# DefaultRui/VLN-VER

Hardware: AMD Instinct MI355X
Metric: viewpoints/sec (multi-view->voxel fwd+bwd), vocc.py config (higher is better)
Workload: dtype bf16

## Files before the change

vln-ver_amd/csrc/ver_gemm.hip:

```cpp
#include "ver_gemm_tile.h"

namespace {
using namespace gemm_tile;
constexpr int kStageBytes = 32768;
constexpr int kStages = 4;
constexpr int kLdsBytes = kStages * kStageBytes;

struct TapArgs {
    const __bf16* lattice;
    long lattice_bytes;
    int B, H, W, C, ntaps, P;
    const float* rowpos;
    const __bf16* cst;
    long cst_bytes;
    int CW, ncst;
    unsigned desc[64];
    long plane_elems;
};

struct GemmArgs {
    const __bf16* A;
    const __bf16* W;
    const float* bias;
    __bf16* C;
// ... 31 lines not shown
    asm volatile("s_load_dword %0, %1, %2" : "=s"(v) : "s"(ts.tab), "s"(idx * 4) : "memory");
    return v;
}
__device__ __forceinline__ void desc_ready(unsigned& d) { asm volatile("s_waitcnt lgkmcnt(0)" : "+s"(d) : : "memory"); }

template <int L>
__device__ __forceinline__ void tap_begin(const TapArgs& t, TapLane& tl, TapWave& ts, unsigned d, __amdgpu_buffer_rsrc_t& ra,
                                          __amdgpu_buffer_rsrc_t rcst) {
    const bool live = ts.tap < t.ntaps;
    const bool is_cst = live && (d >> 31) != 0;
    const int dx = (int)(d << 24) >> 24, dy = (int)(d << 16) >> 24, dz = (int)(d >> 16) & 63, pl = (int)(d >> 22) & 63;
    int o1 = kOutside, o2 = kOutside, seglen = 2 * t.C;
    if (is_cst) {
        seglen = 2 * t.CW;
        if (tl.b1 >= 0) o1 = (tl.pos1 * t.ncst + dz) * t.CW * 2 + tl.chunk;
        if (tl.b2 >= 0) o2 = (tl.pos2 * t.ncst + dz) * t.CW * 2 + tl.chunk;
        ra = rcst;
    } else if (live) {
        const LatticeGeom geom = {t.B, t.H, t.W, t.C};
        const int c1 = cell_off<L>(geom, tl.b1, tl.zl1, tl.y1 + dy, tl.x1 + dx, dz);
        const int c2 = cell_off<L>(geom, tl.b2, tl.zl2, tl.y2 + dy, tl.x2 + dx, dz);
        if (c1 != kOutside) o1 = c1 + tl.chunk;
        if (c2 != kOutside) o2 = c2 + tl.chunk;
        ra = __builtin_amdgcn_make_buffer_rsrc((void*)(t.lattice + (long)pl * t.plane_elems), 0,
                                               (int)max(0L, min(t.lattice_bytes, 0x7FFFFFFFL)), 0x00020000);
    }
    ts.seglen = seglen;
    tl.vo1 = o1;
    tl.vo2 = o2;
}

template <int IMPL, bool PRO>
__device__ __forceinline__ void request_a(char* dst, const GemmLane& c, __amdgpu_buffer_rsrc_t& ra, __amdgpu_buffer_rsrc_t rcst,
                                          int& soA, const TapArgs& t, TapLane& tl, TapWave& ts) {
    if constexpr (IMPL < 0) {
        __builtin_amdgcn_raw_ptr_buffer_load_lds(ra, (lds_void*)dst, 16, c.voA, soA, 0, 0);
        __builtin_amdgcn_raw_ptr_buffer_load_lds(ra, (lds_void*)(dst + 1024), 16, c.voA, soA + c.stepA16, 0, 0);
        soA += 64;
    } else {
        __builtin_amdgcn_raw_ptr_buffer_load_lds(ra, (lds_void*)dst, 16, tl.vo1, ts.ch, 0, 0);
        __builtin_amdgcn_raw_ptr_buffer_load_lds(ra, (lds_void*)(dst + 1024), 16, tl.vo2, ts.ch, 0, 0);
        ts.ch += 64;
        if (ts.ch == ts.seglen) {
            ts.ch = 0;
            ts.tap += 1;
            const unsigned d = ts.next;
            ts.next = desc_load(ts, min(ts.tap + 1, t.ntaps - 1));
            if constexpr (PRO) desc_ready(ts.next);
            tap_begin<IMPL>(t, tl, ts, d, ra, rcst);
        }
    }
}

template <int ST, int IMPL>
__device__ __forceinline__ void phase(char* lds, f32x4 (&acc)[8][4], const GemmLane& c, __amdgpu_buffer_rsrc_t& ra,
                                      __amdgpu_buffer_rsrc_t rw, int& soA, int& soW, const TapArgs& t, TapLane& tl, TapWave& ts,
                                      __amdgpu_buffer_rsrc_t rcst) {
    constexpr int SB = (ST & 1) * kStageBytes;
    constexpr int UP = ST >= 2 ? 65536 : 0;
    const int a0 = c.offA0 + UP;
    i32x4 av[8];
    i32x2 bl[4], bh[4];
    av[0] = row_read<SB>(a0);
    av[1] = row_read<SB + 1024>(a0);
#pragma unroll
    for (int q = 0; q < 4; ++q) {
        const int b = c.offB[q] + UP;
        bl[q] = tr_read<SB + 16384>(b);
        bh[q] = tr_read<SB + 16384 + 512>(b);
        if (q == 0) av[2] = row_read<SB + 2048>(a0), av[3] = row_read<SB + 3072>(a0);
        if (q == 1) av[4] = row_read<SB + 4096>(a0), av[5] = row_read<SB + 5120>(a0);
        if (q == 2) av[6] = row_read<SB + 6144>(a0), av[7] = row_read<SB + 7168>(a0);
    }
    constexpr int DS = ((ST + 2) % kStages) * kStageBytes;
    request_a<IMPL, false>(lds + DS + c.dmaA, c, ra, rcst, soA, t, tl, ts);
    __builtin_amdgcn_raw_ptr_buffer_load_lds(rw, (lds_void*)(lds + DS + 16384 + c.dmaW), 16, c.voW, soW, 0, 0);
    __builtin_amdgcn_raw_ptr_buffer_load_lds(rw, (lds_void*)(lds + DS + 24576 + c.dmaW), 16, c.voW, soW + c.stepW, 0, 0);
    soW += 2 * c.stepW;
    asm volatile("s_waitcnt vmcnt(4)" ::: "memory");
    __builtin_amdgcn_s_barrier();
    asm volatile("s_waitcnt lgkmcnt(0)"
                 : "+v"(av[0]), "+v"(av[1]), "+v"(av[2]), "+v"(av[3]), "+v"(av[4]), "+v"(av[5]), "+v"(av[6]), "+v"(av[7]), "+v"(bl[0]),
                   "+v"(bh[0]), "+v"(bl[1]), "+v"(bh[1]), "+v"(bl[2]), "+v"(bh[2]), "+v"(bl[3]), "+v"(bh[3])
                 :
                 : "memory");
    if constexpr (IMPL >= 0) asm volatile("" : "+s"(ts.next));
    bf16x8 a[8], b[4];
#pragma unroll
    for (int i = 0; i < 8; ++i) a[i] = __builtin_bit_cast(bf16x8, av[i]);
#pragma unroll
    for (int j = 0; j < 4; ++j) b[j] = frag(bl[j], bh[j]);
    __builtin_amdgcn_sched_barrier(0);
    __builtin_amdgcn_s_setprio(1);
#pragma unroll
    for (int it = 0; it < 8; ++it)
#pragma unroll
        for (int jt = 0; jt < 4; ++jt) acc[it][jt] = __builtin_amdgcn_mfma_f32_16x16x32_bf16(a[it], b[jt], acc[it][jt], 0, 0, 0);
    __builtin_amdgcn_s_setprio(0);
    __builtin_amdgcn_sched_barrier(0);
    __builtin_amdgcn_s_barrier();
}


template <int IMPL>
__global__ __launch_bounds__(512) void k_gemm_nn(GemmArgs p) {
    extern __shared__ __attribute__((aligned(1024))) char lds[];
    const int tid = threadIdx.x, lane = tid & 63;
    const int wave = __builtin_amdgcn_readfirstlane(tid >> 6);
    const int wr = wave >> 2, wc = wave & 3;
    const int item = (int)(blockIdx.x & 7) * p.per_xcd + (int)(blockIdx.x >> 3);
    if ((int)(blockIdx.x >> 3) >= p.per_xcd || item >= p.T * p.S) return;
    const int split = item / p.T, tile = item - split * p.T;
    const int mt = tile / p.tiles_n, nt = tile - mt * p.tiles_n;
    const long row0 = (long)mt * kTile;
    const int k0 = split * p.Kc, klen = min(p.Kc, p.K - k0);
    const int nphase = klen / 32;

    const __bf16* ab = IMPL < 0 ? p.A + row0 * p.lda + k0 : p.t.lattice;
    const long abytes = IMPL < 0 ? ((p.M - row0 - 1) * p.lda + klen) * 2 : p.t.lattice_bytes;
    __amdgpu_buffer_rsrc_t ra = __builtin_amdgcn_make_buffer_rsrc((void*)ab, 0, (int)max(0L, min(abytes, 0xFFFFFFFFL)), 0x00020000);
    const __amdgpu_buffer_rsrc_t rcst = __builtin_amdgcn_make_buffer_rsrc((void*)(IMPL < 0 ? ab : p.t.cst), 0,
                                                                          (int)(IMPL < 0 ? 0L : max(0L, min(p.t.cst_bytes, 0x7FFFFFFFL))), 0x00020000);
    const __bf16* wb = p.W + (long)k0 * p.ldw + (long)nt * kTile;
    const long wbytes = ((long)(klen - 1) * p.ldw + p.N - (long)nt * kTile) * 2;
    const __amdgpu_buffer_rsrc_t rw = __builtin_amdgcn_make_buffer_rsrc((void*)wb, 0, (int)max(0L, min(wbytes, 0xFFFFFFFFL)), 0x00020000);
    GemmLane c;
    {
        const int prow = 32 * wave + (lane >> 2);
        const int pch = (lane & 3) ^ Shape::swz_a(prow & 15);
        c.voA = (int)(prow * p.lda * 2) + pch * 16;
        c.dmaA = wave * 2048;
        c.stepA16 = (int)(16 * p.lda * 2);
        const int wrow = lane >> 3, wch = (lane & 7) ^ Shape::swz(wrow, wave >> 2);
        c.voW = (int)(((8 * (wave >> 2) + wrow) * p.ldw + 64 * (wave & 3)) * 2) + wch * 16;
        c.stepW = (int)(16 * p.ldw * 2);
        c.dmaW = wave * 1024;
    }
    {
        const int lbase = (int)(uintptr_t)(__attribute__((address_space(3))) char*)lds;
        const int i = lane & 15, g = lane >> 4;
        c.offA0 = lbase + (128 * wr + i) * 64 + ((g ^ Shape::swz_a(i)) << 4);
#pragma unroll
        for (int q = 0; q < 4; ++q) {
            const int ch = (2 * q + ((i & 3) >> 1)) ^ Shape::swz(i >> 2, g & 1);
            c.offB[q] = lbase + (g >> 1) * 8192 + (g & 1) * 4096 + (i >> 2) * 128 + ch * 16 + (i & 1) * 8 + wc * 1024;
        }
    }
    TapLane tl = {};
    TapWave ts = {};
    if constexpr (IMPL >= 0) {
        const int prow = 32 * wave + (lane >> 2);
        const int hw = p.t.H * p.t.W;
        auto decode = [&](long r, int& b, int& zl, int& y, int& x) {
            if (r >= p.M) {
                b = -1, zl = y = x = 0;
                return;
            }
            b = (int)(r / p.t.P);
            const int pos = (int)(r - (long)b * p.t.P);
            zl = pos / hw;
            const int rem = pos - zl * hw;
            y = rem / p.t.W;
            x = rem - y * p.t.W;
        };
        decode(row0 + prow, tl.b1, tl.zl1, tl.y1, tl.x1);
        decode(row0 + prow + 16, tl.b2, tl.zl2, tl.y2, tl.x2);
        tl.pos1 = (tl.zl1 * p.t.H + tl.y1) * p.t.W + tl.x1;
        tl.pos2 = (tl.zl2 * p.t.H + tl.y2) * p.t.W + tl.x2;
        tl.chunk = ((lane & 3) ^ Shape::swz_a(prow & 15)) * 16;
        ts.tab = (const __attribute__((address_space(4))) unsigned*)((const __attribute__((address_space(4))) char*)
                     __builtin_amdgcn_kernarg_segment_ptr() + offsetof(GemmArgs, t) + offsetof(TapArgs, desc));
        unsigned d = desc_load(ts, 0);
        desc_ready(d);
        ts.next = desc_load(ts, min(1, p.t.ntaps - 1));
        tap_begin<IMPL>(p.t, tl, ts, d, ra, rcst);
        desc_ready(ts.next);
    }
    Shape::acc_t acc[Shape::NI][Shape::NJ];
#pragma unroll
    for (int it = 0; it < Shape::NI; ++it)
#pragma unroll
        for (int jt = 0; jt < Shape::NJ; ++jt)
#pragma unroll
            for (int r = 0; r < Shape::NR; ++r) acc[it][jt][r] = 0.0f;

    int soA = 0, soW = 0;
#pragma unroll
    for (int s = 0; s < 2; ++s) {
        request_a<IMPL, true>(lds + s * kStageBytes + c.dmaA, c, ra, rcst, soA, p.t, tl, ts);
        __builtin_amdgcn_raw_ptr_buffer_load_lds(rw, (lds_void*)(lds + s * kStageBytes + 16384 + c.dmaW), 16, c.voW, soW, 0, 0);
        __builtin_amdgcn_raw_ptr_buffer_load_lds(rw, (lds_void*)(lds + s * kStageBytes + 24576 + c.dmaW), 16, c.voW, soW + c.stepW, 0, 0);
        soW += 2 * c.stepW;
    }
    asm volatile("s_waitcnt vmcnt(4)" ::: "memory");
    __builtin_amdgcn_s_barrier();
    if (wr == 1) __builtin_amdgcn_s_barrier();

    int s = 0;
    for (; s + kStages <= nphase; s += kStages) {
        phase<0, IMPL>(lds, acc, c, ra, rw, soA, soW, p.t, tl, ts, rcst);
        phase<1, IMPL>(lds, acc, c, ra, rw, soA, soW, p.t, tl, ts, rcst);
        phase<2, IMPL>(lds, acc, c, ra, rw, soA, soW, p.t, tl, ts, rcst);
        phase<3, IMPL>(lds, acc, c, ra, rw, soA, soW, p.t, tl, ts, rcst);
    }
    const int rem = nphase - s;
    if (rem > 0) phase<0, IMPL>(lds, acc, c, ra, rw, soA, soW, p.t, tl, ts, rcst);
    if (rem > 1) phase<1, IMPL>(lds, acc, c, ra, rw, soA, soW, p.t, tl, ts, rcst);
    if (rem > 2) phase<2, IMPL>(lds, acc, c, ra, rw, soA, soW, p.t, tl, ts, rcst);
    if (wr == 0) __builtin_amdgcn_s_barrier();
    asm volatile("s_waitcnt vmcnt(0)" ::: "memory");

    if (p.S > 1) {
        float* out = p.ws + (long)split * p.M * p.N;
        const long i0 = row0 + 128 * wr + Shape::lane_row(lane);
        const int j0 = nt * kTile + 64 * wc + (lane & (Shape::TW - 1));
#pragma unroll
        for (int it = 0; it < Shape::NI; ++it)
#pragma unroll
            for (int jt = 0; jt < Shape::NJ; ++jt) {
                const int j = j0 + Shape::TW * jt;
#pragma unroll
                for (int r = 0; r < Shape::NR; ++r) {
                    const long i = i0 + Shape::TW * it + Shape::reg_row(r);
                    if (i < p.M && j < p.N) out[i * p.N + j] = acc[it][jt][r];
                }
            }
        return;
    }
    __bf16* cb = p.C + row0 * p.ldc + (long)nt * kTile;
    const long cbytes = ((p.M - row0 - 1) * p.ldc + p.N - (long)nt * kTile) * 2;
    const __amdgpu_buffer_rsrc_t rc = __builtin_amdgcn_make_buffer_rsrc((void*)cb, 0, (int)max(0L, min(cbytes, 0xFFFFFFFFL)), 0x00020000);
    const int ldc2 = (int)(p.ldc * 2);
    const int vbase = (128 * wr + Shape::lane_row(lane)) * ldc2 + (64 * wc + (lane & (Shape::TW - 1))) * 2;
    const bool haspos = IMPL >= 0 && p.t.rowpos != nullptr;
    const int pos0 = haspos ? (int)((row0 + 128 * wr + Shape::lane_row(lane)) % p.t.P) : 0;
#pragma unroll
    for (int jt = 0; jt < Shape::NJ; ++jt) {
        const int j = nt * kTile + 64 * wc + Shape::TW * jt + (lane & (Shape::TW - 1));
        const float bj = (p.bias && j < p.N) ? p.bias[j] : 0.0f;
        const int vo = j < p.N ? vbase + 2 * Shape::TW * jt : -2;
#pragma unroll
        for (int it = 0; it < Shape::NI; ++it) {
            float add[Shape::NR];
#pragma unroll
            for (int r = 0; r < Shape::NR; ++r) {
                add[r] = bj;
                if (haspos) {
                    int pp = pos0 + Shape::TW * it + Shape::reg_row(r);
                    while (pp >= p.t.P) pp -= p.t.P;
                    const long row = row0 + 128 * wr + Shape::lane_row(lane) + Shape::TW * it + Shape::reg_row(r);
                    if (j < p.N && row < p.M) add[r] += p.t.rowpos[(long)pp * p.N + j];
                }
            }
#pragma unroll
            for (int r = 0; r < Shape::NR; ++r) {
                const __bf16 v = (__bf16)(acc[it][jt][r] + add[r]);
                __builtin_amdgcn_raw_buffer_store_b16(__builtin_bit_cast(short, v), rc, vo, (Shape::TW * it + Shape::reg_row(r)) * ldc2, 0);
            }
        }
    }
}
// ... 171 lines not shown
```

vln-ver_amd/csrc/ver_wgrad.hip:

```cpp
#include "ver_gemm_tile.h"

namespace {
using namespace gemm_tile;

constexpr int kSlabRows = 16;
constexpr int kSlabBytes = 2 * kSlabRows * kTile * 2;
constexpr int kRing = 8;
constexpr int kLdsBytes = kRing * kSlabBytes;
constexpr int kPhaseSlabs = 2;
constexpr int kAhead = 4;
static_assert(kAhead >= kPhaseSlabs && kAhead + 4 <= kRing, "prefetch distance against the ring (WAR on the slot)");

struct WgradArgs {
    const __bf16* A;
    const __bf16* G;
    float* ws;
    long lda, ldg, M, Mc;
    int S, Ka, N, tiles_n, T;
    void* out;
    long ldo;
    int out_bf16;
    const __bf16* lattice;
    long lattice_bytes;
    const __bf16* cst;
// ... 11 lines not shown
    int tend;
    int rows_left;
    int vo;
    int taddr1, pend1, vo1;
};

template <int L>
__device__ __forceinline__ int wtap_table_entry(const WgradArgs& t, int seg, int pos) {
    if (seg < 0) return kOutside;
    if (t.kind[seg]) return (pos * t.ncst + t.dz[seg]) * t.CW * 2;
    const int hw = t.H * t.W;
    const int zl = pos / hw, rem = pos - zl * hw;
    const int y = rem / t.W, x = rem - y * t.W;
    return cell_off<L>(LatticeGeom{t.B, t.H, t.W, t.C}, 0, zl, y + t.dy[seg], x + t.dx[seg], t.dz[seg]);
}

__device__ __forceinline__ int lds_read_b32(int addr) {
    int v;
    asm volatile("ds_read_b32 %0, %1" : "=v"(v) : "v"(addr) : "memory");
    return v;
}

__device__ __forceinline__ void wtap_step(const WgradArgs& t, WTapLane& tl, int tfetched) {
    tl.boff += tl.pend;
    tl.rows_left -= kSlabRows;
    tl.vo = tl.rows_left > 0 ? (int)((unsigned)tfetched + (unsigned)tl.boff) : kOutside;
    tl.taddr += 4 * kSlabRows;
    tl.pend = 0;
    if (tl.taddr >= tl.tend) tl.taddr -= 4 * t.P, tl.pend = tl.bstep;
}

__device__ __forceinline__ void wtap_step2(const WgradArgs& t, WTapLane& tl, int tfetched0, int tfetched1) {
    tl.boff += tl.pend;
    tl.rows_left -= kSlabRows;
    tl.vo = tl.rows_left > 0 ? (int)((unsigned)tfetched0 + (unsigned)tl.boff) : kOutside;
    tl.boff += tl.pend1;
    tl.rows_left -= kSlabRows;
    tl.vo1 = tl.rows_left > 0 ? (int)((unsigned)tfetched1 + (unsigned)tl.boff) : kOutside;
    tl.taddr = tl.taddr1 + 4 * kSlabRows;
    tl.pend = 0;
    if (tl.taddr >= tl.tend) tl.taddr -= 4 * t.P, tl.pend = tl.bstep;
    tl.taddr1 = tl.taddr + 4 * kSlabRows;
    tl.pend1 = 0;
    if (tl.taddr1 >= tl.tend) tl.taddr1 -= 4 * t.P, tl.pend1 = tl.bstep;
}

struct WgradLane {
    int offA[4], offB[4];
    int voA, voG;
    int stepA, stepG;
    int dmaoff;
};

template <int PS, int IMPL>
__device__ __forceinline__ void phase(char* lds, f32x4 (&acc)[8][4], const WgradLane& c, __amdgpu_buffer_rsrc_t ra,
                                      __amdgpu_buffer_rsrc_t rg, unsigned& soA, unsigned& soG, const WgradArgs& t, WTapLane& tl) {
    constexpr int SB = ((2 * PS) & 3) * kSlabBytes;
    constexpr int UP = 2 * PS >= 4 ? 65536 : 0;
    i32x2 al[8], ah[8], bl[4], bh[4];
    int tn0 = 0, tn1 = 0;
#pragma unroll
    for (int q = 0; q < 4; ++q) {
        const int a = c.offA[q] + UP, b = c.offB[q] + UP;
        al[q] = tr_read<SB>(a);
        ah[q] = tr_read<SB + 512>(a);
        bl[q] = tr_read<SB>(b);
        bh[q] = tr_read<SB + 512>(b);
        al[4 + q] = tr_read<SB + 1024>(a);
        ah[4 + q] = tr_read<SB + 1536>(a);
    }
#pragma unroll
    for (int u = 0; u < 2; ++u) {
        const int ds = (2 * PS + u + kAhead) % kRing;
        if constexpr (IMPL < 0) {
            __builtin_amdgcn_raw_ptr_buffer_load_lds(ra, (lds_void*)(lds + ds * kSlabBytes + c.dmaoff), 16, c.voA, (int)soA, 0, 0);
        } else {
            __builtin_amdgcn_raw_ptr_buffer_load_lds(ra, (lds_void*)(lds + ds * kSlabBytes + c.dmaoff), 16, u ? tl.vo1 : tl.vo, 0, 0, 0);
            if (u) tn1 = lds_read_b32(tl.taddr1);
            else tn0 = lds_read_b32(tl.taddr);
        }
        __builtin_amdgcn_raw_ptr_buffer_load_lds(rg, (lds_void*)(lds + ds * kSlabBytes + kSlabBytes / 2 + c.dmaoff), 16, c.voG, (int)soG, 0, 0);
        soA += (unsigned)c.stepA;
        soG += (unsigned)c.stepG;
    }
    asm volatile("s_waitcnt vmcnt(%0)" ::"n"(2 * (kAhead - kPhaseSlabs)) : "memory");
    __builtin_amdgcn_s_barrier();
    asm volatile("s_waitcnt lgkmcnt(0)"
                 : "+v"(al[0]), "+v"(ah[0]), "+v"(al[1]), "+v"(ah[1]), "+v"(al[2]), "+v"(ah[2]), "+v"(al[3]), "+v"(ah[3]), "+v"(al[4]),
                   "+v"(ah[4]), "+v"(al[5]), "+v"(ah[5]), "+v"(al[6]), "+v"(ah[6]), "+v"(al[7]), "+v"(ah[7]), "+v"(bl[0]), "+v"(bh[0]),
                   "+v"(bl[1]), "+v"(bh[1]), "+v"(bl[2]), "+v"(bh[2]), "+v"(bl[3]), "+v"(bh[3]), "+v"(tn0), "+v"(tn1)
                 :
                 : "memory");
    bf16x8 a[8], b[4];
#pragma unroll
    for (int i = 0; i < 8; ++i) a[i] = frag(al[i], ah[i]);
#pragma unroll
    for (int j = 0; j < 4; ++j) b[j] = frag(bl[j], bh[j]);
    __builtin_amdgcn_sched_barrier(0);
    __builtin_amdgcn_s_setprio(1);
#pragma unroll
    for (int it = 0; it < 8; ++it)
#pragma unroll
        for (int jt = 0; jt < 4; ++jt)
            acc[it][jt] = __builtin_amdgcn_mfma_f32_16x16x32_bf16(a[it], b[jt], acc[it][jt], 0, 0, 0);
    __builtin_amdgcn_s_setprio(0);
    __builtin_amdgcn_sched_barrier(0);
    if constexpr (IMPL >= 0) {
        wtap_step2(t, tl, tn0, tn1);
        __builtin_amdgcn_sched_barrier(0);
    }
    __builtin_amdgcn_s_barrier();
}

template <int PS, int IMPL>
__device__ __forceinline__ void phases_from(int left, char* lds, f32x4 (&acc)[8][4], const WgradLane& c,
                                            __amdgpu_buffer_rsrc_t ra, __amdgpu_buffer_rsrc_t rg, unsigned& soA, unsigned& soG,
                                            const WgradArgs& t, WTapLane& tl) {
    if constexpr (PS < kRing / kPhaseSlabs) {
        if (left > PS * kPhaseSlabs) {
            phase<PS, IMPL>(lds, acc, c, ra, rg, soA, soG, t, tl);
            phases_from<PS + 1, IMPL>(left, lds, acc, c, ra, rg, soA, soG, t, tl);
        }
    }
}

template <int IMPL>
__device__ __forceinline__ void wgrad_body(const WgradArgs& p) {
    extern __shared__ __attribute__((aligned(1024))) char lds[];
    const int tid = threadIdx.x, lane = tid & 63;
    const int wave = __builtin_amdgcn_readfirstlane(tid >> 6);
    const int wr = wave >> 2, wc = wave & 3;
    int chunk, tile;
    {
        const int b = blockIdx.x;
        if ((p.S & 7) == 0) {
            const int xcd = b & 7, idx = b >> 3;
            chunk = xcd + 8 * (idx / p.T);
            tile = idx % p.T;
        } else {
            chunk = b / p.T;
            tile = b % p.T;
        }
    }
    const int mt = tile / p.tiles_n, nt = tile - mt * p.tiles_n;
    const long row0 = (long)chunk * p.Mc;
    const long rows = max(0L, min(p.Mc, p.M - row0));
    const int nslab = (int)((rows + kSlabRows * kPhaseSlabs - 1) / (kSlabRows * kPhaseSlabs)) * kPhaseSlabs;

    const __bf16* ab = IMPL < 0 ? p.A + row0 * p.lda + (long)mt * kTile : nullptr;
    const __bf16* gb = p.G + row0 * p.ldg + (long)nt * kTile;
    const long abytes = ((p.M - row0 - 1) * p.lda + p.Ka - (long)mt * kTile) * 2;
    const long gbytes = ((p.M - row0 - 1) * p.ldg + p.N - (long)nt * kTile) * 2;
    const __amdgpu_buffer_rsrc_t rg = __builtin_amdgcn_make_buffer_rsrc((void*)gb, 0, (int)max(0L, min(gbytes, 0xFFFFFFFFL)), 0x00020000);
    WgradLane c;
    const int prow = lane >> 3, pch = (lane & 7) ^ Shape::swz(prow, wave >> 2);
    WTapLane tl = {};
    bool a_cst = false;
    if constexpr (IMPL >= 0) {
        int* tables = reinterpret_cast<int*>(lds + kLdsBytes);
        auto seg_of = [&](int col0) {
            int seg = -1;
            for (int i = 0; i < p.nseg; ++i)
                if (col0 >= p.seg_start[i] && col0 < p.seg_start[i + 1]) seg = i;
            return seg;
        };
        for (int q = 0; q < 4; ++q) {
            const int seg = seg_of(mt * kTile + 64 * q);
            for (int i = tid; i < p.P; i += 512) tables[q * p.P + i] = wtap_table_entry<IMPL>(p, seg, i);
        }
        __syncthreads();
        const int col0 = mt * kTile + 64 * (wave & 3);
        const int seg = seg_of(col0);
        a_cst = seg >= 0 && p.kind[seg];
        const long r = row0 + 8 * (wave >> 2) + prow;
        const int b0 = (int)(r / p.P), pos0 = (int)(r - (long)b0 * p.P);
        tl.bstep = a_cst ? 0 : (IMPL == 3 ? p.H * p.W : 4 * p.H * p.W) * p.C * 2;
        tl.boff = b0 * tl.bstep + (seg < 0 ? 0 : (col0 - p.seg_start[seg]) * 2) + pch * 16;
        const int lbase = (int)(uintptr_t)(__attribute__((address_space(3))) char*)(lds + kLdsBytes) + (wave & 3) * p.P * 4;
        tl.tend = lbase + 4 * p.P;
        tl.taddr = lbase + 4 * pos0;
        tl.pend = 0;
        tl.rows_left = (int)min(min(p.M, row0 + p.Mc) - r, 0x7FFFFFF0L) + kSlabRows;
        int t0 = lds_read_b32(tl.taddr);
        asm volatile("s_waitcnt lgkmcnt(0)" : "+v"(t0)::"memory");
        wtap_step(p, tl, t0);
    }
    const __amdgpu_buffer_rsrc_t ra =
        IMPL < 0 ? __builtin_amdgcn_make_buffer_rsrc((void*)ab, 0, (int)max(0L, min(abytes, 0xFFFFFFFFL)), 0x00020000)
                 : __builtin_amdgcn_make_buffer_rsrc((void*)(a_cst ? p.cst : p.lattice), 0,
                                                     (int)max(0L, min(a_cst ? p.cst_bytes : p.lattice_bytes, 0x7FFFFFFFL)), 0x00020000);
    c.voA = (int)(((8 * (wave >> 2) + prow) * p.lda + 64 * (wave & 3)) * 2) + pch * 16;
    c.voG = (int)(((8 * (wave >> 2) + prow) * p.ldg + 64 * (wave & 3)) * 2) + pch * 16;
    c.stepA = (int)(kSlabRows * p.lda * 2);
    c.stepG = (int)(kSlabRows * p.ldg * 2);
    c.dmaoff = wave * 1024;
    unsigned soA = 0, soG = 0;

    {
        const int g = lane >> 4, cl = lane & 15;
        const int lbase = (int)(uintptr_t)(__attribute__((address_space(3))) char*)lds;
#pragma unroll
        for (int q = 0; q < 4; ++q) {
            const int ch = (2 * q + ((cl & 3) >> 1)) ^ Shape::swz(cl >> 2, g & 1);
            const int rowoff = lbase + (g >> 1) * kSlabBytes + (g & 1) * 4096 + (cl >> 2) * 128 + ch * 16 + (cl & 1) * 8;
            c.offA[q] = rowoff + 2 * wr * 1024;
            c.offB[q] = rowoff + wc * 1024 + kSlabBytes / 2;
        }
    }

    Shape::acc_t acc[Shape::NI][Shape::NJ];
#pragma unroll
    for (int it = 0; it < Shape::NI; ++it)
#pragma unroll
        for (int jt = 0; jt < Shape::NJ; ++jt)
#pragma unroll
            for (int r = 0; r < Shape::NR; ++r) acc[it][jt][r] = 0.0f;

#pragma unroll
    for (int s = 0; s < kAhead; ++s) {
        if constexpr (IMPL < 0) {
            __builtin_amdgcn_raw_ptr_buffer_load_lds(ra, (lds_void*)(lds + s * kSlabBytes + c.dmaoff), 16, c.voA, (int)soA, 0, 0);
        } else {
            __builtin_amdgcn_raw_ptr_buffer_load_lds(ra, (lds_void*)(lds + s * kSlabBytes + c.dmaoff), 16, tl.vo, 0, 0, 0);
            int tn = lds_read_b32(tl.taddr);
            asm volatile("s_waitcnt lgkmcnt(0)" : "+v"(tn)::"memory");
            wtap_step(p, tl, tn);
        }
        __builtin_amdgcn_raw_ptr_buffer_load_lds(rg, (lds_void*)(lds + s * kSlabBytes + kSlabBytes / 2 + c.dmaoff), 16, c.voG, (int)soG, 0, 0);
        soA += (unsigned)c.stepA;
        soG += (unsigned)c.stepG;
    }
    if constexpr (IMPL >= 0) {
        const int vo0 = tl.vo;
        int tn = lds_read_b32(tl.taddr);
        asm volatile("s_waitcnt lgkmcnt(0)" : "+v"(tn)::"memory");
        wtap_step(p, tl, tn);
        tl.vo1 = tl.vo;
        tl.vo = vo0;
        tl.taddr1 = tl.taddr + 4 * kSlabRows;
        tl.pend1 = 0;
        if (tl.taddr1 >= tl.tend) tl.taddr1 -= 4 * p.P, tl.pend1 = tl.bstep;
    }
    asm volatile("s_waitcnt vmcnt(%0)" ::"n"(2 * (kAhead - kPhaseSlabs)) : "memory");
    __builtin_amdgcn_s_barrier();
    if (wr == 1) __builtin_amdgcn_s_barrier();

    int s = 0;
    for (; s + kRing <= nslab; s += kRing) phases_from<0, IMPL>(kRing, lds, acc, c, ra, rg, soA, soG, p, tl);
    phases_from<0, IMPL>(nslab - s, lds, acc, c, ra, rg, soA, soG, p, tl);
    if (wr == 0) __builtin_amdgcn_s_barrier();
    asm volatile("s_waitcnt vmcnt(0)" ::: "memory");

    const int i0 = mt * kTile + 128 * wr + Shape::lane_row(lane), j0 = nt * kTile + 64 * wc + (lane & (Shape::TW - 1));
    if (p.S == 1 && p.out) {
#pragma unroll
        for (int it = 0; it < Shape::NI; ++it)
#pragma unroll
            for (int jt = 0; jt < Shape::NJ; ++jt) {
                const int j = j0 + Shape::TW * jt;
#pragma unroll
                for (int r = 0; r < Shape::NR; ++r) {
                    const int i = i0 + Shape::TW * it + Shape::reg_row(r);
                    if (i < p.Ka && j < p.N) {
                        if (p.out_bf16)
                            reinterpret_cast<__bf16*>(p.out)[(long)i * p.ldo + j] = (__bf16)acc[it][jt][r];
                        else
                            reinterpret_cast<float*>(p.out)[(long)i * p.ldo + j] = acc[it][jt][r];
                    }
                }
            }
        return;
    }
    float* out = p.ws + (long)chunk * p.Ka * p.N;
#pragma unroll
    for (int it = 0; it < Shape::NI; ++it)
#pragma unroll
        for (int jt = 0; jt < Shape::NJ; ++jt) {
            const int j = j0 + Shape::TW * jt;
#pragma unroll
            for (int r = 0; r < Shape::NR; ++r) {
                const int i = i0 + Shape::TW * it + Shape::reg_row(r);
                if (i < p.Ka && j < p.N) out[(long)i * p.N + j] = acc[it][jt][r];
            }
        }
}

__global__ __launch_bounds__(512) void k_wgrad_tn(WgradArgs p) {
    wgrad_body<-1>(p);
}

template <int L>
__global__ __launch_bounds__(512) void k_wgrad_tn_seg(WgradArgs p) {
    wgrad_body<L>(p);
}

template <typename OT>
__global__ __launch_bounds__(256) void k_wgrad_reduce(const float* __restrict__ ws, OT* __restrict__ out, long ldo, int S,
                                                      int Ka, int N) {
    const long n4 = (long)Ka * N / 4;
    const long stride = (long)Ka * N;
    for (long e = blockIdx.x * 256L + threadIdx.x; e < n4; e += (long)gridDim.x * 256) {
        float4 acc = *reinterpret_cast<const float4*>(ws + 4 * e);
        for (int s = 1; s < S; ++s) {
            const float4 v = *reinterpret_cast<const float4*>(ws + s * stride + 4 * e);
            acc.x += v.x;
            acc.y += v.y;
            acc.z += v.z;
            acc.w += v.w;
        }
        const long i = (4 * e) / N, j = (4 * e) - i * N;
        OT* o = out + i * ldo + j;
        if constexpr (sizeof(OT) == 4) {
            *reinterpret_cast<float4*>(o) = acc;
        } else {
            typedef __bf16 bf16x4 __attribute__((ext_vector_type(4)));
            bf16x4 v;
            v.x = (__bf16)acc.x;
            v.y = (__bf16)acc.y;
            v.z = (__bf16)acc.z;
            v.w = (__bf16)acc.w;
            *reinterpret_cast<bf16x4*>(o) = v;
        }
    }
}

long max_chunk_rows(long ld) {
    if (ld <= 0) return 45000;
    const long rows = (0xFFFFFFFFL / (ld * 2)) - 16 * kRing - 2 * kSlabRows - 1;
    return rows < 45000 ? (rows > 2 * kSlabRows ? rows : 2 * kSlabRows) : 45000;
}

int pick_splits(long M, int Ka, int N, long ld = 0) {
    const long cap = max_chunk_rows(ld);
    const long tiles = (long)((Ka + kTile - 1) / kTile) * ((N + kTile - 1) / kTile);
    static const int cand[] = {1, 2, 3, 4, 6, 8, 12, 16, 24, 32, 48, 64};
    int best = 0;
    double best_us = 0.0;
    for (int s : cand) {
        if ((M + s - 1) / s > cap) continue;
        if (s > 1 && M / s < 256) break;
        if (M > 32768 && s % 8) continue;
        const long rounds = (tiles * s + 255) / 256;
        const double slabs = (double)((M + s - 1) / s + 15) / 16.0;
        double us = (double)rounds * (slabs * 0.37 + 8.0) + (s == 1 ? 0.25 : (double)s) * (double)Ka * (double)N * 8.0 / 3.0e6;
        if (s % 8 == 0) us *= 0.97;
        if (!best || us < best_us) {
// ... 135 lines not shown
```

Before: 758.9.

## Add narrow-tile path for ragged last N tile in GEMM and wgrad kernels

When the final column tile holds at most 64 valid columns (e.g. N=832 = 3×256+64), the GEMM and weight-gradient kernels now go to a narrow variant. In it, all eight waves split the tile's rows and each wave computes only NI=2 row fragments over one 64-column strip. This avoids issuing MFMAs and LDS reads for columns that are entirely out of bounds on the edge tile. The cost is a second code path with different LDS offset and wave mapping, which raises correctness risk and code size. A scratch A/B microbenchmark script is also added.

Measured after the change: 762.5, median of 6. About the same (+0.5%).

```diff
diff --git a/scratch/gemm_edge_tiles_ab.py b/scratch/gemm_edge_tiles_ab.py
--- /dev/null
+++ b/scratch/gemm_edge_tiles_ab.py
@@ -0,0 +1,121 @@
+import argparse
+import ctypes
+import json
+import os
+import shutil
+import statistics
+import sys
+import tempfile
+
+import torch
+
+KA = 4480
+c_long, c_int, c_void = ctypes.c_long, ctypes.c_int, ctypes.c_void_p
+
+
+def load(path):
+    L = ctypes.CDLL(path)
+    L.ver_gemm_nn.argtypes = [c_void, c_long, c_void, c_long, c_void, c_void, c_long, c_long, c_int, c_int, c_int, c_void]
+    L.ver_wgrad_tn.argtypes = [c_void, c_long, c_void, c_long, c_long, c_int, c_int, c_void, c_long, c_int, c_int, c_int, c_void,
+                               c_long, c_void]
+    L.ver_wgrad_tn_splits_ld.argtypes = [c_long, c_int, c_int, c_long]
+    L.ver_wgrad_tn_workspace.argtypes = [c_long, c_int, c_int, c_int]
+    L.ver_wgrad_tn_workspace.restype = c_long
+    return L
+
+
+def timed(f, n=6):
+    for _ in range(2):
+        f()
+    torch.cuda.synchronize()
+    a, b = torch.cuda.Event(enable_timing=True), torch.cuda.Event(enable_timing=True)
+    a.record()
+    for _ in range(n):
+        f()
+    b.record()
+    torch.cuda.synchronize()
+    return a.elapsed_time(b) / n
+
+
+def main():
+    ap = argparse.ArgumentParser()
+    ap.add_argument('parent')
+    ap.add_argument('new')
+    ap.add_argument('--reps', type=int, default=5)
+    ap.add_argument('--rows', type=int, default=552960)
+    ap.add_argument('--out', default=None)
+    args = ap.parse_args()
+    M = args.rows
+    tmp = tempfile.mkdtemp()
+    copy = shutil.copy(args.parent, os.path.join(tmp, 'libver_hip_parent_copy.so'))
+    arms = [('parent', load(args.parent)), ('new', load(args.new)), ('parent_copy', load(copy))]
+    dev = 'cuda'
+    st = torch.cuda.current_stream().cuda_stream
+    out = open(args.out, 'a') if args.out else None
+
+    def emit(rec):
+        line = json.dumps(rec)
+        print(line, flush=True)
+        if out:
+            out.write(line + '\n')
+            out.flush()
+
+    def check(rc, what):
+        if rc != 0:
+            sys.exit('%s returned %d' % (what, rc))
+
+    emit(dict(kind='arms', parent=os.path.basename(args.parent), new=os.path.basename(args.new), rows=M, Ka=KA, widths=[832, 768],
+              operands='N(0,1)', order='parent, new, parent copy, %d times over, one process' % args.reps))
+    torch.manual_seed(0)
+    rand = lambda *s: torch.randn(*s, device=dev).bfloat16()
+    big = rand(M, KA)
+    med = {}
+    for fam in ('gemm_nn', 'wgrad_tn'):
+        for N in (832, 768):
+            small = rand(KA, N) if fam == 'gemm_nn' else rand(M, N)
+            res = torch.empty((M, N) if fam == 'gemm_nn' else (KA, N), dtype=torch.bfloat16, device=dev)
+            s = arms[0][1].ver_wgrad_tn_splits_ld(M, KA, N, KA)
+            nb = arms[0][1].ver_wgrad_tn_workspace(M, KA, N, s)
+            ws = torch.empty(nb // 4, dtype=torch.float32, device=dev)
+
+            def run(L):
+                if fam == 'gemm_nn':
+                    check(L.ver_gemm_nn(big.data_ptr(), KA, small.data_ptr(), N, None, res.data_ptr(), N, M, KA, N, 0, st), fam)
+                else:
+                    assert L.ver_wgrad_tn_splits_ld(M, KA, N, KA) == s
+                    check(L.ver_wgrad_tn(big.data_ptr(), KA, small.data_ptr(), N, M, KA, N, res.data_ptr(), N, 1, s, 0, ws.data_ptr(),
+                                         nb, st), fam)
+
+            got = {}
+            for name, L in arms[:2]:
+                res.zero_()
+                run(L)
+                got[name] = res.clone()
+            emit(dict(kind='bit_identity', family=fam, N=N, new_equals_parent=bool(torch.equal(got['parent'], got['new'])),
+                      result_abs_max=float(got['parent'].float().abs().max())))
+            del got
+            samples = {name: [] for name, _ in arms}
+            for _ in range(args.reps):
+                for name, L in arms:
+                    samples[name].append(timed(lambda: run(L)))
+            fl = 2.0 * M * KA * N
+            for name, _ in arms:
+                med[fam, N, name] = statistics.median(samples[name])
+                emit(dict(kind='microbench', family=fam, arm=name, M=M, K=KA, N=N, splits=s if fam == 'wgrad_tn' else 1,
+                          ms=[round(x, 4) for x in samples[name]], ms_median=round(med[fam, N, name], 4),
+                          tflops=round(fl / med[fam, N, name] / 1e9, 1)))
+            spread = abs(med[fam, N, 'parent'] - med[fam, N, 'parent_copy'])
+            gain = med[fam, N, 'parent'] - med[fam, N, 'new']
+            emit(dict(kind='verdict', family=fam, N=N, parent_ms=round(med[fam, N, 'parent'], 4), new_ms=round(med[fam, N, 'new'], 4),
+                      parent_aa_spread_ms=round(spread, 4), gain_ms=round(gain, 4),
+                      speedup=round(med[fam, N, 'parent'] / med[fam, N, 'new'], 4), clears_twice_the_spread=bool(gain > 2 * spread)))
+            del small, res, ws
+        for name, _ in arms:
+            t832, t768 = med[fam, 832, name], med[fam, 768, name]
+            emit(dict(kind='narrow_tile_cost', family=fam, arm=name, t832_ms=round(t832, 4), t768_ms=round(t768, 4),
+                      fraction_of_a_full_tile=round((t832 - t768) / (t768 / 3.0), 3)))
+    shutil.rmtree(tmp, ignore_errors=True)
+
+
+if __name__ == '__main__':
+    main()
diff --git a/vln-ver_amd/csrc/ver_gemm.hip b/vln-ver_amd/csrc/ver_gemm.hip
--- a/vln-ver_amd/csrc/ver_gemm.hip
+++ b/vln-ver_amd/csrc/ver_gemm.hip
@@ -107,14 +107,14 @@
     }
 }
 
-template <int ST, int IMPL>
-__device__ __forceinline__ void phase(char* lds, f32x4 (&acc)[8][4], const GemmLane& c, __amdgpu_buffer_rsrc_t& ra,
+template <int ST, int IMPL, int NI>
+__device__ __forceinline__ void phase(char* lds, f32x4 (&acc)[NI][4], const GemmLane& c, __amdgpu_buffer_rsrc_t& ra,
                                       __amdgpu_buffer_rsrc_t rw, int& soA, int& soW, const TapArgs& t, TapLane& tl, TapWave& ts,
                                       __amdgpu_buffer_rsrc_t rcst) {
     constexpr int SB = (ST & 1) * kStageBytes;
     constexpr int UP = ST >= 2 ? 65536 : 0;
     const int a0 = c.offA0 + UP;
-    i32x4 av[8];
+    i32x4 av[NI];
     i32x2 bl[4], bh[4];
     av[0] = row_read<SB>(a0);
     av[1] = row_read<SB + 1024>(a0);
@@ -123,9 +123,11 @@
         const int b = c.offB[q] + UP;
         bl[q] = tr_read<SB + 16384>(b);
         bh[q] = tr_read<SB + 16384 + 512>(b);
-        if (q == 0) av[2] = row_read<SB + 2048>(a0), av[3] = row_read<SB + 3072>(a0);
-        if (q == 1) av[4] = row_read<SB + 4096>(a0), av[5] = row_read<SB + 5120>(a0);
-        if (q == 2) av[6] = row_read<SB + 6144>(a0), av[7] = row_read<SB + 7168>(a0);
+        if constexpr (NI == 8) {
+            if (q == 0) av[2] = row_read<SB + 2048>(a0), av[3] = row_read<SB + 3072>(a0);
+            if (q == 1) av[4] = row_read<SB + 4096>(a0), av[5] = row_read<SB + 5120>(a0);
+            if (q == 2) av[6] = row_read<SB + 6144>(a0), av[7] = row_read<SB + 7168>(a0);
+        }
     }
     constexpr int DS = ((ST + 2) % kStages) * kStageBytes;
     request_a<IMPL, false>(lds + DS + c.dmaA, c, ra, rcst, soA, t, tl, ts);
@@ -134,21 +136,28 @@
     soW += 2 * c.stepW;
     asm volatile("s_waitcnt vmcnt(4)" ::: "memory");
     __builtin_amdgcn_s_barrier();
-    asm volatile("s_waitcnt lgkmcnt(0)"
-                 : "+v"(av[0]), "+v"(av[1]), "+v"(av[2]), "+v"(av[3]), "+v"(av[4]), "+v"(av[5]), "+v"(av[6]), "+v"(av[7]), "+v"(bl[0]),
-                   "+v"(bh[0]), "+v"(bl[1]), "+v"(bh[1]), "+v"(bl[2]), "+v"(bh[2]), "+v"(bl[3]), "+v"(bh[3])
-                 :
-                 : "memory");
+    if constexpr (NI == 8)
+        asm volatile("s_waitcnt lgkmcnt(0)"
+                     : "+v"(av[0]), "+v"(av[1]), "+v"(av[2]), "+v"(av[3]), "+v"(av[4]), "+v"(av[5]), "+v"(av[6]), "+v"(av[7]), "+v"(bl[0]),
+                       "+v"(bh[0]), "+v"(bl[1]), "+v"(bh[1]), "+v"(bl[2]), "+v"(bh[2]), "+v"(bl[3]), "+v"(bh[3])
+                     :
+                     : "memory");
+    else
+        asm volatile("s_waitcnt lgkmcnt(0)"
+                     : "+v"(av[0]), "+v"(av[1]), "+v"(bl[0]), "+v"(bh[0]), "+v"(bl[1]), "+v"(bh[1]), "+v"(bl[2]), "+v"(bh[2]), "+v"(bl[3]),
+                       "+v"(bh[3])
+                     :
+                     : "memory");
     if constexpr (IMPL >= 0) asm volatile("" : "+s"(ts.next));
-    bf16x8 a[8], b[4];
-#pragma unroll
-    for (int i = 0; i < 8; ++i) a[i] = __builtin_bit_cast(bf16x8, av[i]);
+    bf16x8 a[NI], b[4];
+#pragma unroll
+    for (int i = 0; i < NI; ++i) a[i] = __builtin_bit_cast(bf16x8, av[i]);
 #pragma unroll
     for (int j = 0; j < 4; ++j) b[j] = frag(bl[j], bh[j]);
     __builtin_amdgcn_sched_barrier(0);
     __builtin_amdgcn_s_setprio(1);
 #pragma unroll
-    for (int it = 0; it < 8; ++it)
+    for (int it = 0; it < NI; ++it)
 #pragma unroll
         for (int jt = 0; jt < 4; ++jt) acc[it][jt] = __builtin_amdgcn_mfma_f32_16x16x32_bf16(a[it], b[jt], acc[it][jt], 0, 0, 0);
     __builtin_amdgcn_s_setprio(0);
@@ -156,6 +165,118 @@
     __builtin_amdgcn_s_barrier();
 }
 
+
+constexpr int kNarrowNI = 2;
+constexpr int kNarrowCols = Shape::NJ * Shape::TW;
+static_assert(8 * kNarrowNI * Shape::TW == kTile, "eight waves cover the tile's rows");
+
+__device__ __forceinline__ void gemm_narrow_tile(const GemmArgs& p, int split, int mt, int nt) {
+    extern __shared__ __attribute__((aligned(1024))) char lds[];
+    const int tid = threadIdx.x, lane = tid & 63;
+    const int wave = __builtin_amdgcn_readfirstlane(tid >> 6);
+    const int rbase = 16 * kNarrowNI * wave;
+    const long row0 = (long)mt * kTile;
+    const int k0 = split * p.Kc, klen = min(p.Kc, p.K - k0);
+    const int nphase = klen / 32;
+    const __bf16* ab = p.A + row0 * p.lda + k0;
+    const long abytes = ((p.M - row0 - 1) * p.lda + klen) * 2;
+    __amdgpu_buffer_rsrc_t ra = __builtin_amdgcn_make_buffer_rsrc((void*)ab, 0, (int)max(0L, min(abytes, 0xFFFFFFFFL)), 0x00020000);
+    const __amdgpu_buffer_rsrc_t rcst = __builtin_amdgcn_make_buffer_rsrc((void*)ab, 0, 0, 0x00020000);
+    const __bf16* wb = p.W + (long)k0 * p.ldw + (long)nt * kTile;
+    const long wbytes = ((long)(klen - 1) * p.ldw + p.N - (long)nt * kTile) * 2;
+    const __amdgpu_buffer_rsrc_t rw = __builtin_amdgcn_make_buffer_rsrc((void*)wb, 0, (int)max(0L, min(wbytes, 0xFFFFFFFFL)), 0x00020000);
+    GemmLane c;
+    {
+        const int prow = 32 * wave + (lane >> 2);
+        const int pch = (lane & 3) ^ Shape::swz_a(prow & 15);
+        c.voA = (int)(prow * p.lda * 2) + pch * 16;
+        c.dmaA = wave * 2048;
+        c.stepA16 = (int)(16 * p.lda * 2);
+        const int wrow = lane >> 3, wch = (lane & 7) ^ Shape::swz(wrow, wave >> 2);
+        c.voW = (int)(((8 * (wave >> 2) + wrow) * p.ldw + 64 * (wave & 3)) * 2) + wch * 16;
+        c.stepW = (int)(16 * p.ldw * 2);
+        c.dmaW = wave * 1024;
+        const int lbase = (int)(uintptr_t)(__attribute__((address_space(3))) char*)lds;
+        const int i = lane & 15, g = lane >> 4;
+        c.offA0 = lbase + (rbase + i) * 64 + ((g ^ Shape::swz_a(i)) << 4);
+#pragma unroll
+        for (int q = 0; q < 4; ++q) {
+            const int ch = (2 * q + ((i & 3) >> 1)) ^ Shape::swz(i >> 2, g & 1);
+            c.offB[q] = lbase + (g >> 1) * 8192 + (g & 1) * 4096 + (i >> 2) * 128 + ch * 16 + (i & 1) * 8;
+        }
+    }
+    TapLane tl = {};
+    TapWave ts = {};
+    Shape::acc_t acc[kNarrowNI][Shape::NJ];
+#pragma unroll
+    for (int it = 0; it < kNarrowNI; ++it)
+#pragma unroll
+        for (int jt = 0; jt < Shape::NJ; ++jt)
+#pragma unroll
+            for (int r = 0; r < Shape::NR; ++r) acc[it][jt][r] = 0.0f;
+
+    int soA = 0, soW = 0;
+#pragma unroll
+    for (int s = 0; s < 2; ++s) {
+        request_a<-1, true>(lds + s * kStageBytes + c.dmaA, c, ra, rcst, soA, p.t, tl, ts);
+        __builtin_amdgcn_raw_ptr_buffer_load_lds(rw, (lds_void*)(lds + s * kStageBytes + 16384 + c.dmaW), 16, c.voW, soW, 0, 0);
+        __builtin_amdgcn_raw_ptr_buffer_load_lds(rw, (lds_void*)(lds + s * kStageBytes + 24576 + c.dmaW), 16, c.voW, soW + c.stepW, 0, 0);
+        soW += 2 * c.stepW;
+    }
+    asm volatile("s_waitcnt vmcnt(4)" ::: "memory");
+    __builtin_amdgcn_s_barrier();
+    if (wave >> 2) __builtin_amdgcn_s_barrier();
+
+    int s = 0;
+    for (; s + kStages <= nphase; s += kStages) {
+        phase<0, -1, kNarrowNI>(lds, acc, c, ra, rw, soA, soW, p.t, tl, ts, rcst);
+        phase<1, -1, kNarrowNI>(lds, acc, c, ra, rw, soA, soW, p.t, tl, ts, rcst);
+        phase<2, -1, kNarrowNI>(lds, acc, c, ra, rw, soA, soW, p.t, tl, ts, rcst);
+        phase<3, -1, kNarrowNI>(lds, acc, c, ra, rw, soA, soW, p.t, tl, ts, rcst);
+    }
+    const int rem = nphase - s;
+    if (rem > 0) phase<0, -1, kNarrowNI>(lds, acc, c, ra, rw, soA, soW, p.t, tl, ts, rcst);
+    if (rem > 1) phase<1, -1, kNarrowNI>(lds, acc, c, ra, rw, soA, soW, p.t, tl, ts, rcst);
+    if (rem > 2) phase<2, -1, kNarrowNI>(lds, acc, c, ra, rw, soA, soW, p.t, tl, ts, rcst);
+    if ((wave >> 2) == 0) __builtin_amdgcn_s_barrier();
+    asm volatile("s_waitcnt vmcnt(0)" ::: "memory");
+
+    const int col = lane & (Shape::TW - 1);
+    if (p.S > 1) {
+        float* out = p.ws + (long)split * p.M * p.N;
+        const long i0 = row0 + rbase + Shape::lane_row(lane);
+#pragma unroll
+        for (int it = 0; it < kNarrowNI; ++it)
+#pragma unroll
+            for (int jt = 0; jt < Shape::NJ; ++jt) {
+                const int j = nt * kTile + Shape::TW * jt + col;
+#pragma unroll
+                for (int r = 0; r < Shape::NR; ++r) {
+                    const long i = i0 + Shape::TW * it + Shape::reg_row(r);
+                    if (i < p.M && j < p.N) out[i * p.N + j] = acc[it][jt][r];
+                }
+            }
+        return;
+    }
+    __bf16* cb = p.C + row0 * p.ldc + (long)nt * kTile;
+    const long cbytes = ((p.M - row0 - 1) * p.ldc + p.N - (long)nt * kTile) * 2;
+    const __amdgpu_buffer_rsrc_t rc = __builtin_amdgcn_make_buffer_rsrc((void*)cb, 0, (int)max(0L, min(cbytes, 0xFFFFFFFFL)), 0x00020000);
+    const int ldc2 = (int)(p.ldc * 2);
+    const int vbase = (rbase + Shape::lane_row(lane)) * ldc2 + col * 2;
+#pragma unroll
+    for (int jt = 0; jt < Shape::NJ; ++jt) {
+        const int j = nt * kTile + Shape::TW * jt + col;
+        const float bj = (p.bias && j < p.N) ? p.bias[j] : 0.0f;
+        const int vo = j < p.N ? vbase + 2 * Shape::TW * jt : -2;
+#pragma unroll
+        for (int it = 0; it < kNarrowNI; ++it)
+#pragma unroll
+            for (int r = 0; r < Shape::NR; ++r) {
+                const __bf16 v = (__bf16)(acc[it][jt][r] + bj);
+                __builtin_amdgcn_raw_buffer_store_b16(__builtin_bit_cast(short, v), rc, vo, (Shape::TW * it + Shape::reg_row(r)) * ldc2, 0);
+            }
+    }
+}
 
 template <int IMPL>
 __global__ __launch_bounds__(512) void k_gemm_nn(GemmArgs p) {
@@ -167,6 +288,12 @@
     if ((int)(blockIdx.x >> 3) >= p.per_xcd || item >= p.T * p.S) return;
     const int split = item / p.T, tile = item - split * p.T;
     const int mt = tile / p.tiles_n, nt = tile - mt * p.tiles_n;
+    if constexpr (IMPL < 0) {
+        if (nt == p.tiles_n - 1 && p.N - kTile * nt <= kNarrowCols) {
+            gemm_narrow_tile(p, split, mt, nt);
+            return;
+        }
+    }
     const long row0 = (long)mt * kTile;
     const int k0 = split * p.Kc, klen = min(p.Kc, p.K - k0);
     const int nphase = klen / 32;
@@ -253,15 +380,15 @@
 
     int s = 0;
     for (; s + kStages <= nphase; s += kStages) {
-        phase<0, IMPL>(lds, acc, c, ra, rw, soA, soW, p.t, tl, ts, rcst);
-        phase<1, IMPL>(lds, acc, c, ra, rw, soA, soW, p.t, tl, ts, rcst);
-        phase<2, IMPL>(lds, acc, c, ra, rw, soA, soW, p.t, tl, ts, rcst);
-        phase<3, IMPL>(lds, acc, c, ra, rw, soA, soW, p.t, tl, ts, rcst);
+        phase<0, IMPL, Shape::NI>(lds, acc, c, ra, rw, soA, soW, p.t, tl, ts, rcst);
+        phase<1, IMPL, Shape::NI>(lds, acc, c, ra, rw, soA, soW, p.t, tl, ts, rcst);
+        phase<2, IMPL, Shape::NI>(lds, acc, c, ra, rw, soA, soW, p.t, tl, ts, rcst);
+        phase<3, IMPL, Shape::NI>(lds, acc, c, ra, rw, soA, soW, p.t, tl, ts, rcst);
     }
     const int rem = nphase - s;
-    if (rem > 0) phase<0, IMPL>(lds, acc, c, ra, rw, soA, soW, p.t, tl, ts, rcst);
-    if (rem > 1) phase<1, IMPL>(lds, acc, c, ra, rw, soA, soW, p.t, tl, ts, rcst);
-    if (rem > 2) phase<2, IMPL>(lds, acc, c, ra, rw, soA, soW, p.t, tl, ts, rcst);
+    if (rem > 0) phase<0, IMPL, Shape::NI>(lds, acc, c, ra, rw, soA, soW, p.t, tl, ts, rcst);
+    if (rem > 1) phase<1, IMPL, Shape::NI>(lds, acc, c, ra, rw, soA, soW, p.t, tl, ts, rcst);
+    if (rem > 2) phase<2, IMPL, Shape::NI>(lds, acc, c, ra, rw, soA, soW, p.t, tl, ts, rcst);
     if (wr == 0) __builtin_amdgcn_s_barrier();
     asm volatile("s_waitcnt vmcnt(0)" ::: "memory");
 
diff --git a/vln-ver_amd/csrc/ver_wgrad.hip b/vln-ver_amd/csrc/ver_wgrad.hip
--- a/vln-ver_amd/csrc/ver_wgrad.hip
+++ b/vln-ver_amd/csrc/ver_wgrad.hip
@@ -87,22 +87,29 @@
     int dmaoff;
 };
 
-template <int PS, int IMPL>
-__device__ __forceinline__ void phase(char* lds, f32x4 (&acc)[8][4], const WgradLane& c, __amdgpu_buffer_rsrc_t ra,
+template <int PS, int IMPL, int NI>
+__device__ __forceinline__ void phase(char* lds, f32x4 (&acc)[NI][4], const WgradLane& c, __amdgpu_buffer_rsrc_t ra,
                                       __amdgpu_buffer_rsrc_t rg, unsigned& soA, unsigned& soG, const WgradArgs& t, WTapLane& tl) {
     constexpr int SB = ((2 * PS) & 3) * kSlabBytes;
     constexpr int UP = 2 * PS >= 4 ? 65536 : 0;
-    i32x2 al[8], ah[8], bl[4], bh[4];
+    i32x2 al[NI], ah[NI], bl[4], bh[4];
     int tn0 = 0, tn1 = 0;
 #pragma unroll
     for (int q = 0; q < 4; ++q) {
         const int a = c.offA[q] + UP, b = c.offB[q] + UP;
-        al[q] = tr_read<SB>(a);
-        ah[q] = tr_read<SB + 512>(a);
+        if constexpr (NI == 8) {
+            al[q] = tr_read<SB>(a);
+            ah[q] = tr_read<SB + 512>(a);
+        } else if (q < 2) {
+            al[q & 1] = tr_read<SB>(a);
+            ah[q & 1] = tr_read<SB + 512>(a);
+        }
         bl[q] = tr_read<SB>(b);
         bh[q] = tr_read<SB + 512>(b);
-        al[4 + q] = tr_read<SB + 1024>(a);
-        ah[4 + q] = tr_read<SB + 1536>(a);
+        if constexpr (NI == 8) {
+            al[4 + q] = tr_read<SB + 1024>(a);
+            ah[4 + q] = tr_read<SB + 1536>(a);
+        }
     }
 #pragma unroll
     for (int u = 0; u < 2; ++u) {
@@ -120,21 +127,28 @@
     }
     asm volatile("s_waitcnt vmcnt(%0)" ::"n"(2 * (kAhead - kPhaseSlabs)) : "memory");
     __builtin_amdgcn_s_barrier();
-    asm volatile("s_waitcnt lgkmcnt(0)"
-                 : "+v"(al[0]), "+v"(ah[0]), "+v"(al[1]), "+v"(ah[1]), "+v"(al[2]), "+v"(ah[2]), "+v"(al[3]), "+v"(ah[3]), "+v"(al[4]),
-                   "+v"(ah[4]), "+v"(al[5]), "+v"(ah[5]), "+v"(al[6]), "+v"(ah[6]), "+v"(al[7]), "+v"(ah[7]), "+v"(bl[0]), "+v"(bh[0]),
-                   "+v"(bl[1]), "+v"(bh[1]), "+v"(bl[2]), "+v"(bh[2]), "+v"(bl[3]), "+v"(bh[3]), "+v"(tn0), "+v"(tn1)
-                 :
-                 : "memory");
-    bf16x8 a[8], b[4];
-#pragma unroll
-    for (int i = 0; i < 8; ++i) a[i] = frag(al[i], ah[i]);
+    if constexpr (NI == 8)
+        asm volatile("s_waitcnt lgkmcnt(0)"
+                     : "+v"(al[0]), "+v"(ah[0]), "+v"(al[1]), "+v"(ah[1]), "+v"(al[2]), "+v"(ah[2]), "+v"(al[3]), "+v"(ah[3]), "+v"(al[4]),
+                       "+v"(ah[4]), "+v"(al[5]), "+v"(ah[5]), "+v"(al[6]), "+v"(ah[6]), "+v"(al[7]), "+v"(ah[7]), "+v"(bl[0]), "+v"(bh[0]),
+                       "+v"(bl[1]), "+v"(bh[1]), "+v"(bl[2]), "+v"(bh[2]), "+v"(bl[3]), "+v"(bh[3]), "+v"(tn0), "+v"(tn1)
+                     :
+                     : "memory");
+    else
+        asm volatile("s_waitcnt lgkmcnt(0)"
+                     : "+v"(al[0]), "+v"(ah[0]), "+v"(al[1]), "+v"(ah[1]), "+v"(bl[0]), "+v"(bh[0]), "+v"(bl[1]), "+v"(bh[1]), "+v"(bl[2]),
+                       "+v"(bh[2]), "+v"(bl[3]), "+v"(bh[3]), "+v"(tn0), "+v"(tn1)
+                     :
+                     : "memory");
+    bf16x8 a[NI], b[4];
+#pragma unroll
+    for (int i = 0; i < NI; ++i) a[i] = frag(al[i], ah[i]);
 #pragma unroll
     for (int j = 0; j < 4; ++j) b[j] = frag(bl[j], bh[j]);
     __builtin_amdgcn_sched_barrier(0);
     __builtin_amdgcn_s_setprio(1);
 #pragma unroll
-    for (int it = 0; it < 8; ++it)
+    for (int it = 0; it < NI; ++it)
 #pragma unroll
         for (int jt = 0; jt < 4; ++jt)
             acc[it][jt] = __builtin_amdgcn_mfma_f32_16x16x32_bf16(a[it], b[jt], acc[it][jt], 0, 0, 0);
@@ -147,19 +161,23 @@
     __builtin_amdgcn_s_barrier();
 }
 
-template <int PS, int IMPL>
-__device__ __forceinline__ void phases_from(int left, char* lds, f32x4 (&acc)[8][4], const WgradLane& c,
+template <int PS, int IMPL, int NI>
+__device__ __forceinline__ void phases_from(int left, char* lds, f32x4 (&acc)[NI][4], const WgradLane& c,
                                             __amdgpu_buffer_rsrc_t ra, __amdgpu_buffer_rsrc_t rg, unsigned& soA, unsigned& soG,
                                             const WgradArgs& t, WTapLane& tl) {
     if constexpr (PS < kRing / kPhaseSlabs) {
         if (left > PS * kPhaseSlabs) {
-            phase<PS, IMPL>(lds, acc, c, ra, rg, soA, soG, t, tl);
-            phases_from<PS + 1, IMPL>(left, lds, acc, c, ra, rg, soA, soG, t, tl);
-        }
-    }
-}
-
-template <int IMPL>
+            phase<PS, IMPL, NI>(lds, acc, c, ra, rg, soA, soG, t, tl);
+            phases_from<PS + 1, IMPL, NI>(left, lds, acc, c, ra, rg, soA, soG, t, tl);
+        }
+    }
+}
+
+constexpr int kNarrowNI = 2;
+constexpr int kNarrowCols = Shape::NJ * Shape::TW;
+static_assert(8 * kNarrowNI * Shape::TW == kTile, "eight waves cover the tile's A columns");
+
+template <int IMPL, int NI>
 __device__ __forceinline__ void wgrad_body(const WgradArgs& p) {
     extern __shared__ __attribute__((aligned(1024))) char lds[];
     const int tid = threadIdx.x, lane = tid & 63;
@@ -178,6 +196,7 @@
         }
     }
     const int mt = tile / p.tiles_n, nt = tile - mt * p.tiles_n;
+    const int rbase = NI == Shape::NI ? 128 * wr : 16 * NI * wave, cbase = NI == Shape::NI ? 64 * wc : 0;
     const long row0 = (long)chunk * p.Mc;
     const long rows = max(0L, min(p.Mc, p.M - row0));
     const int nslab = (int)((rows + kSlabRows * kPhaseSlabs - 1) / (kSlabRows * kPhaseSlabs)) * kPhaseSlabs;
@@ -234,18 +253,21 @@
     {
         const int g = lane >> 4, cl = lane & 15;
         const int lbase = (int)(uintptr_t)(__attribute__((address_space(3))) char*)lds;
+        auto rowoff = [&](int q) {
+            const int ch = (2 * q + ((cl & 3) >> 1)) ^ Shape::swz(cl >> 2, g & 1);
+            return lbase + (g >> 1) * kSlabBytes + (g & 1) * 4096 + (cl >> 2) * 128 + ch * 16 + (cl & 1) * 8;
+        };
 #pragma unroll
         for (int q = 0; q < 4; ++q) {
-            const int ch = (2 * q + ((cl & 3) >> 1)) ^ Shape::swz(cl >> 2, g & 1);
-            const int rowoff = lbase + (g >> 1) * kSlabBytes + (g & 1) * 4096 + (cl >> 2) * 128 + ch * 16 + (cl & 1) * 8;
-            c.offA[q] = rowoff + 2 * wr * 1024;
-            c.offB[q] = rowoff + wc * 1024 + kSlabBytes / 2;
-        }
-    }
-
-    Shape::acc_t acc[Shape::NI][Shape::NJ];
-#pragma unroll
-    for (int it = 0; it < Shape::NI; ++it)
+            const int ta = (rbase >> 4) + (q & 1);
+            c.offA[q] = NI == Shape::NI ? rowoff(q) + 2 * wr * 1024 : rowoff(ta & 3) + (ta >> 2) * 1024;
+            c.offB[q] = rowoff(q) + (cbase >> 6) * 1024 + kSlabBytes / 2;
+        }
+    }
+
+    Shape::acc_t acc[NI][Shape::NJ];
+#pragma unroll
+    for (int it = 0; it < NI; ++it)
 #pragma unroll
         for (int jt = 0; jt < Shape::NJ; ++jt)
 #pragma unroll
@@ -281,15 +303,15 @@
     if (wr == 1) __builtin_amdgcn_s_barrier();
 
     int s = 0;
-    for (; s + kRing <= nslab; s += kRing) phases_from<0, IMPL>(kRing, lds, acc, c, ra, rg, soA, soG, p, tl);
-    phases_from<0, IMPL>(nslab - s, lds, acc, c, ra, rg, soA, soG, p, tl);
+    for (; s + kRing <= nslab; s += kRing) phases_from<0, IMPL, NI>(kRing, lds, acc, c, ra, rg, soA, soG, p, tl);
+    phases_from<0, IMPL, NI>(nslab - s, lds, acc, c, ra, rg, soA, soG, p, tl);
     if (wr == 0) __builtin_amdgcn_s_barrier();
     asm volatile("s_waitcnt vmcnt(0)" ::: "memory");
 
-    const int i0 = mt * kTile + 128 * wr + Shape::lane_row(lane), j0 = nt * kTile + 64 * wc + (lane & (Shape::TW - 1));
+    const int i0 = mt * kTile + rbase + Shape::lane_row(lane), j0 = nt * kTile + cbase + (lane & (Shape::TW - 1));
     if (p.S == 1 && p.out) {
 #pragma unroll
-        for (int it = 0; it < Shape::NI; ++it)
+        for (int it = 0; it < NI; ++it)
 #pragma unroll
             for (int jt = 0; jt < Shape::NJ; ++jt) {
                 const int j = j0 + Shape::TW * jt;
@@ -308,7 +330,7 @@
     }
     float* out = p.ws + (long)chunk * p.Ka * p.N;
 #pragma unroll
-    for (int it = 0; it < Shape::NI; ++it)
+    for (int it = 0; it < NI; ++it)
 #pragma unroll
         for (int jt = 0; jt < Shape::NJ; ++jt) {
             const int j = j0 + Shape::TW * jt;
@@ -321,12 +343,17 @@
 }
 
 __global__ __launch_bounds__(512) void k_wgrad_tn(WgradArgs p) {
-    wgrad_body<-1>(p);
+    const int b = blockIdx.x;
+    const int nt = (((p.S & 7) == 0 ? b >> 3 : b) % p.T) % p.tiles_n;
+    if (nt == p.tiles_n - 1 && p.N - kTile * nt <= kNarrowCols)
+        wgrad_body<-1, kNarrowNI>(p);
+    else
+        wgrad_body<-1, Shape::NI>(p);
 }
 
 template <int L>
 __global__ __launch_bounds__(512) void k_wgrad_tn_seg(WgradArgs p) {
-    wgrad_body<L>(p);
+    wgrad_body<L, Shape::NI>(p);
 }
 
 template <typename OT>
```
